# WeijingShi/Point-GNN

Hardware: AMD Instinct MI355X
Metric: KITTI-shaped frames/sec (car_auto_T3 inference: graph build + GNN, 20000 pts/frame, mean E1 602k) (higher is better)
Workload: dtype f32

## Files before the change

point-gnn_amd/csrc/edge_ws.h:

```cpp
#pragma once
#include "mlp_engine.h"
#include "ws_partition.h"

namespace pgnn {

#ifndef PGNN_WS_SCHED
#define PGNN_WS_SCHED 2
#endif

constexpr int kWsWaves = 8;
constexpr int kWsSchedInts = 2 + kWsMaxSlices * kWsMaxGroups;
constexpr int kWsStampTiles = 38;
constexpr int kWsStampStride = 8 + 4 * kWsStampTiles;

struct EdgeWsArgs {
  const float *P, *Q;
  int ldv4;
  const int32_t *edges;
  int64_t n_edges;
  const int32_t *n_dev;
  const float *wp;
  int nt;
  int relu_from;
  float *out;
  int64_t ldo;
  int num_segments;
  int sorted;
  int xcds;
  int prio;
  long long *ts;
  int32_t *sched;
  int pool_pct;
  int chunk;
  int groups;
  int tile0[kWsMaxGroups + 1];
  int wg0[kWsMaxGroups + 1];
  int balanced;
  int n_wg[kWsMaxGroups];
  short swg0[kWsMaxSlices][kWsMaxGroups + 1];
  short sbase[kWsMaxSlices][kWsMaxGroups];
  float *rows_out;
  int64_t ld_rows;
  float *h1_out;
  const int32_t *nv_dev;
};

__device__ __forceinline__ float opaque_inf() {
  float inf;
  asm("v_mov_b32 %0, 0x7f800000" : "=v"(inf));
  return inf;
}
__device__ __forceinline__ float max_nc(float a, float b, float inf) {
  return __builtin_amdgcn_fmed3f(a, b, inf);
}

typedef float v2f __attribute__((ext_vector_type(2)));
__device__ __forceinline__ v2f pk_sub(v2f a, v2f b) {
  v2f d;
  asm("v_pk_add_f32 %0, %1, %2 neg_lo:[0,1] neg_hi:[0,1]"
      : "=v"(d)
      : "v"(a), "v"(b));
  return d;
}

template <int CTRL>
__device__ __forceinline__ float dpp_mov(float x) {
  return __int_as_float(
      __builtin_amdgcn_update_dpp(0, __float_as_int(x), CTRL, 0xF, 0xF, false));
}

template <int NTG>
__device__ __forceinline__ float ws_v(const v4f (&v)[NTG], int i) {
  return i < 4 * NTG ? v[i >> 2][i & 3] : kFloatLowest;
}

template <int NTG, class ARGS>
__device__ __forceinline__ void ws_flush(const ARGS &a, const float *bias_lds,
                                         int t0, int lane, int d,
                                         const v4f (&v)[NTG], bool whole,
                                         float inf) {
  if (d < 0 || d >= a.num_segments) return;
  int zero;
  asm volatile("s_mov_b32 %0, 0" : "=s"(zero));
  const int n = (lane & 15) + zero, g = lane >> 4;
  const bool b0 = n & 1, b1 = n & 2, b2 = n & 4, b3 = n & 8;
  float A[16], B[8], C[4], D[2];
#pragma unroll
  for (int j = 0; j < 16; ++j) {
    if (2 * j < 4 * NTG) {
      const float x0 = ws_v<NTG>(v, 2 * j), x1 = ws_v<NTG>(v, 2 * j + 1);
      A[j] = max_nc(b0 ? x1 : x0, dpp_mov<0xB1>(b0 ? x0 : x1), inf);
    } else {
      A[j] = kFloatLowest;
    }
  }
#pragma unroll
  for (int k = 0; k < 8; ++k)
    B[k] = max_nc(b1 ? A[2 * k + 1] : A[2 * k],
                  dpp_mov<0x4E>(b1 ? A[2 * k] : A[2 * k + 1]), inf);
#pragma unroll
  for (int l = 0; l < 4; ++l)
    C[l] = max_nc(b2 ? B[2 * l + 1] : B[2 * l],
                  __shfl_xor(b2 ? B[2 * l] : B[2 * l + 1], 4), inf);
#pragma unroll
  for (int m = 0; m < 2; ++m)
    D[m] = max_nc(b3 ? C[2 * m + 1] : C[2 * m],
                  __shfl_xor(b3 ? C[2 * m] : C[2 * m + 1], 8), inf);
  float *orow = a.out + (int64_t)d * a.ldo + 16 * t0;
#pragma unroll
  for (int m = 0; m < 2; ++m) {
    const int i = 16 * m + n;
    if (i < 4 * NTG) {
      const int c = 16 * (i >> 2) + 4 * g + (i & 3);
      float x = D[m] + bias_lds[c];
      if (16 * t0 + c >= a.relu_from) x = x > 0.0f ? x : 0.0f;
      if (whole)
        orow[c] = x;
      else
        atomic_max_f32(orow + c, x + 0.0f);
    }
  }
}

struct WsRun {
  int cur_d;
  bool left_closed;
  bool has;
};

template <int NTG, class ARGS>
__device__ __forceinline__ void ws_epilogue(const ARGS &a, const float *bias_lds,
                                            int t0, int lane,
                                            const v4f (&acc)[NTG],
                                            v4f (&carry)[NTG], unsigned starts,
                                            int my_d, WsRun &st, bool fin,
                                            int d_after, float inf) {
  const int n = lane & 15;
  int cur_d = st.cur_d;
  bool cur_left_closed = st.left_closed, cur_has = st.has;
  int pos = 0;
  if (!(starts & 1u)) {
    const int f = starts ? __builtin_ctz(starts) : 16;
    if (f == 16) {
#pragma unroll
      for (int t = 0; t < NTG; ++t)
#pragma unroll
        for (int r = 0; r < 4; ++r)
          carry[t][r] = max_nc(carry[t][r], acc[t][r], inf);
    } else {
      const bool in_run = n < f;
#pragma unroll
      for (int t = 0; t < NTG; ++t)
#pragma unroll
        for (int r = 0; r < 4; ++r)
          carry[t][r] =
              max_nc(carry[t][r], in_run ? acc[t][r] : kFloatLowest, inf);
    }
    cur_has = true;
    pos = f;
  }
  while (pos < 16) {
    if (cur_has)
      ws_flush<NTG>(a, bias_lds, t0, lane, cur_d, carry,
                    a.sorted && cur_left_closed &&
                        (!fin || d_after != cur_d),
                    inf);
    if (fin) break;
    const unsigned rest = starts & ~((2u << pos) - 1u);
    const int nextpos = rest ? __builtin_ctz(rest) : 16;
    const bool in_run = n >= pos && n < nextpos;
#pragma unroll
    for (int t = 0; t < NTG; ++t)
#pragma unroll
      for (int r = 0; r < 4; ++r)
        carry[t][r] = in_run ? acc[t][r] : kFloatLowest;
    cur_d = __builtin_amdgcn_readlane(my_d, pos);
    cur_left_closed = true;
    cur_has = true;
    pos = nextpos;
  }
  st.cur_d = cur_d;
  st.left_closed = cur_left_closed;
  st.has = cur_has;
}

}

#include "ws_sum.h"

namespace pgnn {

template <int KQ, int NTG, bool EMIT, bool ROWS = false, class POL = WsMax>
__device__ __forceinline__ void edge_ws_body(const EdgeWsArgs &a,
                                             const v4f *__restrict__ wl, int t0,
                                             const float *bias_lds,
                                             int64_t tile_first,
                                             int64_t tile_last, int lane,
                                             long long *tsw, int &stamped,
                                             const int64_t E) {
  if (tile_first >= tile_last) return;
  const int n = lane & 15;
  const int64_t e_first = tile_first * 16;
  const int64_t e_end = tile_last * 16 < E ? tile_last * 16 : E;
  const v4f *__restrict__ P4 = reinterpret_cast<const v4f *>(a.P);
  const v4f *__restrict__ Q4 = reinterpret_cast<const v4f *>(a.Q);
  const int2 *__restrict__ e2 = reinterpret_cast<const int2 *>(a.edges);

  int cur_d = e_first > 0 ? a.edges[2 * (e_first - 1) + 1] : -1;
  int d_after = e_end < E ? a.edges[2 * e_end + 1] : -1;
  cur_d = __builtin_amdgcn_readfirstlane(cur_d);
  d_after = __builtin_amdgcn_readfirstlane(d_after);
  bool cur_left_closed = false, cur_has = false;
  constexpr float kIdentity = POL::kSum ? 0.0f : kFloatLowest;
  v4f carry[NTG];
#pragma unroll
  for (int t = 0; t < NTG; ++t)
    carry[t] = (v4f){kIdentity, kIdentity, kIdentity, kIdentity};

  const float inf = opaque_inf();
  bool nxt_ok = e_first + n < E;
  int2 nxt = e2[nxt_ok ? e_first + n : 0];
  for (int64_t tile = tile_first;; ++tile) {
    const bool fin = tile >= tile_last;
    const int64_t e0 = tile * 16;
    if (a.prio) __builtin_amdgcn_s_setprio(3);
    int lz;
    asm volatile("v_mov_b32 %0, %1" : "=v"(lz) : "v"(lane));
    const int g = lz >> 4;
    int lz1 = lz + 64 * 64, lz2 = lz + 128 * 64;
    asm volatile("" : "+v"(lz1));
    asm volatile("" : "+v"(lz2));
    const v4f *__restrict__ wfrag[3] = {wl + lz, wl + lz1, wl + lz2};
    long long *tst = nullptr;
    if (tsw && stamped < kWsStampTiles) tst = tsw + 8 + 4 * stamped++;
    if (tst) {
      __builtin_amdgcn_sched_barrier(0);
      const long long c = __builtin_readcyclecounter();
      if (lane == 0) tst[0] = c;
      __builtin_amdgcn_sched_barrier(0);
    }
    v4f acc[NTG];
    unsigned starts = 1u;
    int my_d = -1;
    if (fin) {
#pragma unroll
      for (int t = 0; t < NTG; ++t) acc[t] = (v4f){0.f, 0.f, 0.f, 0.f};
    } else {
    [[maybe_unused]] const int my_s = nxt_ok ? nxt.x : 0;
    my_d = nxt_ok ? nxt.y : -1;
    nxt_ok = tile + 1 < tile_last && e0 + 16 + n < E;
    nxt = e2[nxt_ok ? e0 + 16 + n : 0];
    v4f in[KQ];
    if constexpr (ROWS) {
      const int64_t row = e0 + n < E ? e0 + n : 0;
      const v4f *__restrict__ hr = P4 + row * a.ldv4 + g;
#pragma unroll
      for (int q = 0; q < KQ; ++q) in[q] = hr[4 * q];
      __builtin_amdgcn_sched_barrier(0);
    } else {
      const int dq = ((unsigned)my_d < (unsigned)a.num_segments) ? my_d : 0;
      const v4f *__restrict__ pr = P4 + (int64_t)my_s * a.ldv4 + g;
      const v4f *__restrict__ qr = Q4 + (int64_t)dq * a.ldv4 + g;
      v4f pq[KQ];
#pragma unroll
      for (int q = 0; q < KQ; ++q) {
#ifdef PGNN_WS_ABL_NO_GATHER
        in[q] = pr[0];
        pq[q] = qr[0];
#else
        in[q] = pr[4 * q];
        pq[q] = qr[4 * q];
#endif
      }
      __builtin_amdgcn_sched_barrier(0);
#pragma unroll
      for (int q = 0; q < KQ; ++q) {
        const v2f lo = pk_sub((v2f){in[q][0], in[q][1]}, (v2f){pq[q][0], pq[q][1]});
        const v2f hi = pk_sub((v2f){in[q][2], in[q][3]}, (v2f){pq[q][2], pq[q][3]});
        in[q][0] = max_nc(lo[0], 0.0f, inf);
        in[q][1] = max_nc(lo[1], 0.0f, inf);
        in[q][2] = max_nc(hi[0], 0.0f, inf);
        in[q][3] = max_nc(hi[1], 0.0f, inf);
      }
    }
    if constexpr (EMIT) {
      if (a.h1_out && t0 == 0 && e0 + n < E) {
        v4f *hrow = reinterpret_cast<v4f *>(a.h1_out) + (e0 + n) * a.ldv4 + g;
#pragma unroll
        for (int q = 0; q < KQ; ++q) hrow[4 * q] = in[q];
      }
    }
    __builtin_amdgcn_sched_barrier(0);
    if (tst) {
      const long long c = __builtin_readcyclecounter();
      if (lane == 0) tst[1] = c;
      __builtin_amdgcn_sched_barrier(0);
    }
    __builtin_amdgcn_s_setprio(0);
    {
      v4f w[2][NTG];
#pragma unroll
      for (int t = 0; t < NTG; ++t) {
        acc[t] = (v4f){0.f, 0.f, 0.f, 0.f};
        w[0][t] = wfrag[0][t * 64];
      }
      __builtin_amdgcn_sched_barrier(0);
#pragma unroll
      for (int q = 0; q < KQ; ++q) {
        __builtin_amdgcn_s_waitcnt(0xC07F);
        __builtin_amdgcn_sched_barrier(0);
        if (q + 1 < KQ) {
#pragma unroll
          for (int t = 0; t < NTG; ++t)
#ifdef PGNN_WS_ABL_NO_LDS
            w[(q + 1) & 1][t] = w[q & 1][t];
#else
            w[(q + 1) & 1][t] = wfrag[((q + 1) * NTG + t) >> 6]
                                     [(((q + 1) * NTG + t) & 63) * 64];
#endif
        }
#pragma unroll
        for (int s = 0; s < 4; ++s)
#pragma unroll
          for (int t = 0; t < NTG; ++t)
            acc[t] = __builtin_amdgcn_mfma_f32_16x16x4f32(
                w[q & 1][t][s], in[q][s], acc[t], 0, 0, 0);
#if PGNN_WS_SCHED == 2
#pragma unroll
        for (int t = 0; t < NTG; ++t) {
          __builtin_amdgcn_sched_group_barrier(0x8 , 3, 0);
          if (q + 1 < KQ)
            __builtin_amdgcn_sched_group_barrier(0x100 , 1, 0);
        }
        __builtin_amdgcn_sched_group_barrier(0x8 , NTG, 0);
#else
        if (q + 1 < KQ)
          __builtin_amdgcn_sched_group_barrier(0x100 , NTG, 0);
        __builtin_amdgcn_sched_group_barrier(0x8 , 4 * NTG, 0);
#endif
        __builtin_amdgcn_sched_barrier(0);
      }
    }
    if (tst) {
      const long long c = __builtin_readcyclecounter();
      if (lane == 0) tst[2] = c;
      __builtin_amdgcn_sched_barrier(0);
    }
    if constexpr (EMIT) {
      const int64_t row = e0 + n;
      if (row < E) {
        float *dstp = a.rows_out + row * a.ld_rows + 16 * t0 + 4 * g;
#pragma unroll
        for (int t = 0; t < NTG; ++t) {
          const v4f bb = *reinterpret_cast<const v4f *>(bias_lds + 16 * t + 4 * g);
          v4f y;
#pragma unroll
          for (int r = 0; r < 4; ++r) {
            float x = acc[t][r] + bb[r];
            if (16 * (t0 + t) + 4 * g + r >= a.relu_from) x = x > 0.0f ? x : 0.0f;
            y[r] = x;
          }
          *reinterpret_cast<v4f *>(dstp + 16 * t) = y;
        }
      }
    }
    if (a.prio) __builtin_amdgcn_s_setprio(3);
    const int up = __shfl_up(my_d, 1);
    const int prev = n == 0 ? cur_d : up;
    starts = (unsigned)(__ballot(my_d != prev) & 0xFFFFull);
    }
    WsRun st = {cur_d, cur_left_closed, cur_has};
    if constexpr (POL::kSum)
      ws_epilogue_sum<NTG>(a, bias_lds, t0, lane, acc, carry, starts, my_d, st,
                           fin, d_after, inf);
    else
      ws_epilogue<NTG>(a, bias_lds, t0, lane, acc, carry, starts, my_d, st, fin,
                       d_after, inf);
    cur_d = st.cur_d;
    cur_left_closed = st.left_closed;
    cur_has = st.has;
    if (fin) break;
    if (tst) {
      __builtin_amdgcn_sched_barrier(0);
      const long long c = __builtin_readcyclecounter();
      if (lane == 0) tst[3] = c;
    }
  }
  __builtin_amdgcn_s_setprio(0);
}


struct WsWho {
  int grp, t0, ntg;
  int64_t wi, nw;
};
__device__ __forceinline__ WsWho ws_who_balanced(const EdgeWsArgs &a, int slice,
                                                 int local, int wave) {
  int grp = 0;
  while (grp + 1 < a.groups && local >= a.swg0[slice][grp + 1]) ++grp;
  WsWho w;
  w.grp = grp;
  w.t0 = a.tile0[grp];
  w.ntg = a.tile0[grp + 1] - w.t0;
  w.nw = (int64_t)a.n_wg[grp] * kWsWaves;
  w.wi = (int64_t)(a.sbase[slice][grp] + local - a.swg0[slice][grp]) * kWsWaves +
         wave;
  return w;
}


template <int PER, class V, class ARGS, class MAP>
__device__ __forceinline__ void ws_stage(const ARGS &a, V *wl, int n_frag,
                                         MAP src_frag, size_t bias_at, int t0,
                                         int ntg, float *bias_lds, int wave,
                                         int lane) {
  const V *src = reinterpret_cast<const V *>(a.wp);
  V tmp[PER];
#pragma unroll
  for (int i = 0; i < PER; ++i) {
    const int f = wave + i * kWsWaves;
    tmp[i] = src[src_frag(f < n_frag ? f : 0) * 64 + lane];
  }
  __builtin_amdgcn_sched_barrier(0);
#pragma unroll
  for (int i = 0; i < PER; ++i) {
    const int f = wave + i * kWsWaves;
    if (f < n_frag) wl[(size_t)f * 64 + lane] = tmp[i];
  }
  if ((int)threadIdx.x < 16 * ntg)
    bias_lds[threadIdx.x] = a.wp[bias_at + 16 * t0 + threadIdx.x];
}

__device__ __forceinline__ int64_t ws_edge_count(int64_t cap,
                                                 const int32_t *n_dev) {
  if (n_dev) {
    const int64_t nd = *n_dev;
    cap = nd < cap ? nd : cap;
  }
  return cap;
}

__device__ __forceinline__ int ws_group(const EdgeWsArgs &a, int slice,
                                        int local, int wave) {
  if (a.balanced) return ws_who_balanced(a, slice, local, wave).grp;
  int grp = 0;
  while (grp + 1 < a.groups && local >= a.wg0[grp + 1]) ++grp;
  return grp;
}

struct WsShare {
  int64_t first, last, nw, wi;
};
__device__ __forceinline__ WsShare ws_share(const EdgeWsArgs &a, int grp,
                                            int slice, int local, int wave,
                                            int64_t n_wt) {
  WsShare s;
  s.first = n_wt * slice / a.xcds;
  s.last = n_wt * (slice + 1) / a.xcds;
  s.nw = (int64_t)(a.wg0[grp + 1] - a.wg0[grp]) * kWsWaves;
  s.wi = (int64_t)(local - a.wg0[grp]) * kWsWaves + wave;
  if (a.balanced) {
    const WsWho w = ws_who_balanced(a, slice, local, wave);
    s.first = 0;
    s.last = n_wt;
    s.nw = w.nw;
    s.wi = w.wi;
  }
  return s;
}

__device__ __forceinline__ int64_t ws_pool_size(int64_t span, const int32_t *sched,
                                                int pool_pct, int least,
                                                int64_t nw) {
  int64_t pool = sched ? span * pool_pct / 100 : 0;
  if (span - pool < least * nw) pool = 0;
  return pool;
}

__device__ __forceinline__ int ws_pool_claim(int32_t *counter, int chunk,
                                             int lane) {
  int c = 0;
  if (lane == 0)
    c = __hip_atomic_fetch_add(counter, chunk, __ATOMIC_RELAXED,
                               __HIP_MEMORY_SCOPE_AGENT);
  return __builtin_amdgcn_readfirstlane(c);
}

__device__ __forceinline__ void ws_pool_rearm(int32_t *sched, int n_counters,
                                              int lane) {
  if (sched && lane == 0) {
    const int total = (int)gridDim.x * kWsWaves;
    const int done = __hip_atomic_fetch_add(&sched[1], 1, __ATOMIC_ACQ_REL,
                                            __HIP_MEMORY_SCOPE_AGENT);
    if (done == total - 1) {
      for (int i = 0; i < n_counters; ++i)
        __hip_atomic_store(&sched[2 + i], 0, __ATOMIC_RELAXED,
                           __HIP_MEMORY_SCOPE_AGENT);
      __hip_atomic_store(&sched[1], 0, __ATOMIC_RELEASE,
                         __HIP_MEMORY_SCOPE_AGENT);
    }
  }
}

template <int KQ, int NTMAX, bool EMIT = false, bool ROWS = false,
          class POL = WsMax>
__global__ __launch_bounds__(64 * kWsWaves) void edge_ws_kernel(EdgeWsArgs a) {
  extern __shared__ __attribute__((aligned(16))) char smem[];
  v4f *wl = reinterpret_cast<v4f *>(smem);
  float *bias_lds = reinterpret_cast<float *>(wl + KQ * NTMAX * 64);
  const int lane = threadIdx.x & 63;
  const int wave = __builtin_amdgcn_readfirstlane(threadIdx.x >> 6);
  const int slice = blockIdx.x % a.xcds;
  const int local = blockIdx.x / a.xcds;
  const long long rt_entry = a.ts ? (long long)__builtin_amdgcn_s_memrealtime() : 0;
  const int grp = ws_group(a, slice, local, wave);
  const int t0 = a.tile0[grp];
  const int ntg = a.tile0[grp + 1] - t0;
  {
    const v4f *__restrict__ src = reinterpret_cast<const v4f *>(a.wp);
    constexpr int PER = (KQ * NTMAX + kWsWaves - 1) / kWsWaves;
    const int n_frag = KQ * ntg;
    v4f tmp[PER];
#pragma unroll
    for (int i = 0; i < PER; ++i) {
      const int f = wave + i * kWsWaves;
      const int fc = f < n_frag ? f : 0;
      const int q = fc / ntg, t = fc - q * ntg;
      tmp[i] = src[((size_t)q * a.nt + t0 + t) * 64 + lane];
    }
    __builtin_amdgcn_sched_barrier(0);
#pragma unroll
    for (int i = 0; i < PER; ++i) {
      const int f = wave + i * kWsWaves;
      if (f < n_frag) wl[(size_t)f * 64 + lane] = tmp[i];
    }
    if ((int)threadIdx.x < 16 * ntg)
      bias_lds[threadIdx.x] =
          a.wp[(size_t)KQ * a.nt * 256 + 16 * t0 + threadIdx.x];
  }
  __syncthreads();
  const int64_t n_edges = ws_edge_count(a.n_edges, a.n_dev);
  const WsShare s = ws_share(a, grp, slice, local, wave, (n_edges + 15) / 16);
  int64_t span = s.last - s.first;
  const int64_t pool = ws_pool_size(span, a.sched, a.pool_pct, 4, s.nw);
  span -= pool;
  const int64_t pool_first = s.first + span;
  int64_t tile_first = s.first + span * s.wi / s.nw;
  int64_t tile_last = s.first + span * (s.wi + 1) / s.nw;
  long long *tsw = nullptr;
  if (a.ts) {
    tsw = a.ts + ((int64_t)blockIdx.x * kWsWaves + wave) * kWsStampStride;
    if (lane == 0) {
      tsw[0] = __builtin_readcyclecounter();
      tsw[2] = __builtin_amdgcn_s_memrealtime();
      tsw[4] = tile_last - tile_first;
      tsw[5] = ntg + 100 * slice;
      tsw[6] = rt_entry;
    }
  }
  int stamped = 0;
  int32_t *counter = a.sched ? a.sched + 2 + slice * kWsMaxGroups + grp : nullptr;
  for (;;) {
    if (ntg == NTMAX)
      edge_ws_body<KQ, NTMAX, EMIT, ROWS, POL>(a, wl, t0, bias_lds, tile_first,
                                          tile_last, lane, tsw, stamped,
                                          n_edges);
    else
      edge_ws_body<KQ, NTMAX - 1, EMIT, ROWS, POL>(a, wl, t0, bias_lds, tile_first,
                                              tile_last, lane, tsw, stamped,
                                              n_edges);
    if (pool == 0) break;
    const int c = ws_pool_claim(counter, a.chunk, lane);
    if (c >= pool) break;
    tile_first = pool_first + c;
    tile_last = tile_first + a.chunk < s.last ? tile_first + a.chunk : s.last;
  }
  if (tsw && lane == 0) {
    tsw[1] = __builtin_readcyclecounter();
    tsw[3] = __builtin_amdgcn_s_memrealtime();
    tsw[7] = stamped;
  }
  if (a.sched && lane == 0) {
    const int total = (int)gridDim.x * kWsWaves;
    const int done = __hip_atomic_fetch_add(&a.sched[1], 1, __ATOMIC_ACQ_REL,
                                            __HIP_MEMORY_SCOPE_AGENT);
    if (done == total - 1) {
      for (int i = 0; i < a.xcds * kWsMaxGroups; ++i)
        __hip_atomic_store(&a.sched[2 + i], 0, __ATOMIC_RELAXED,
                           __HIP_MEMORY_SCOPE_AGENT);
      __hip_atomic_store(&a.sched[1], 0, __ATOMIC_RELEASE,
                         __HIP_MEMORY_SCOPE_AGENT);
    }
  }
}

}
```

point-gnn_amd/csrc/gnn.hip:

```cpp
#include <atomic>

#include "mlp_engine.h"
#include "edge_ws.h"
#include "edge_ws_split.h"
#include "pool_ws.h"
#include "pool_split.h"
#include "pool_ws_f16.h"

namespace pgnn {
int g_mlp_blocks_per_cu = 4;
int g_edge_msub = 0;
int g_pool_msub = 0;
int g_mlp_pool_pct = 12;
int g_ws_xcds = 8;
int g_ws_prio = 1;
int g_f16_pool = 1;
int g_b16_force = 0;
int g_ws_pool_pct = 0;
int g_ws_chunk = 2;
int g_ws_balance = 1;
int g_ws_reserve = 0;
void *g_mlp_ts = nullptr;
int g_mlp_debug = 0;
}
// ... 1988 lines not shown
  }
  a.c = c;
  a.xyz = xyz;
  a.wx = wx;
  a.n = n_vertices;
  a.n_dev = dk.dev;
  a.P = P;
  a.Q = Q;
  a.ld_pq = ld_pq;
  a.agg = agg;
  a.ld_agg = ld_agg;
  a.ld_tile = lds_ld(16 * pl.kq);
  a.ld_scratch = scratch_ld;
  return 0;
}

int pre_edge_impl(
    const float *h, int64_t ld_h, int32_t c, const float *xyz,
    const pgnn_fc_layer *offset_layers, int32_t n_offset_layers,
    const pgnn_fc_layer *p_layer, const float *wx, int64_t n_vertices, float *P,
    float *Q, int64_t ld_pq, float *agg, int64_t ld_agg, hipStream_t stream,
    const Dyn &dk) {
  PGNN_REQUIRE(n_vertices >= 0 && c > 0 && ld_h >= c && n_offset_layers >= 0 &&
                   n_offset_layers <= PGNN_MAX_LAYERS && p_layer,
               PGNN_E_INVALID, "vertex_pre_edge: bad argument");
  if (n_vertices == 0) return 0;
  PGNN_REQUIRE(h && xyz && wx && P && Q && (!agg || ld_agg > 0), PGNN_E_INVALID,
               "vertex_pre_edge: null pointer");
  ChainDev off;
  LayerDev pl;
  PreEdgeArgs a;
  const int rc = plan_pre_edge("vertex_pre_edge", c, xyz, offset_layers,
                               n_offset_layers, p_layer, wx, n_vertices, P, Q,
                               ld_pq, agg, ld_agg, dk, 0, off, pl, a);
  if (rc) return rc;
  a.h = h;
  a.ld_h = ld_h;
  const size_t lds =
      (size_t)16 * (a.ld_tile + a.ld_scratch + lds_ld(16 * pl.nt)) * 4;
  PGNN_REQUIRE(lds <= 160 * 1024, PGNN_E_UNSUPPORTED,
               "vertex_pre_edge: layer too wide for the LDS tile");
  g_vertex_lds[0][dk.dev ? 1 : 0] = (int64_t)lds;
  return launch_lds(
      dk.dev ? vertex_pre_edge_kernel<true> : vertex_pre_edge_kernel<false>,
      dim3((unsigned)dyn_grid_tiles(dk, n_vertices)), dim3(64 * kRowsWaves), lds,
      stream, off, pl, a);
}
}

namespace {
int plan_front(const float *x, int64_t ld_x, int32_t nx,
               const pgnn_fc_layer *front_layers, int32_t n_front,
               const float *residual, int64_t ld_res, float *y, int64_t ld_y,
               Plan &pf, FrontArgs &f) {
  PGNN_REQUIRE(x && y && nx > 0 && ld_x >= nx, PGNN_E_INVALID,
               "fused vertex stage: bad front input");
  int rc = make_plan(front_layers, n_front, nx, pf);
  if (rc) return rc;
  const int nt_last = pf.chain.l[n_front - 1].nt;
  PGNN_REQUIRE(nt_last <= kMaxTilesPerPass, PGNN_E_UNSUPPORTED,
               "fused vertex stage: front chain wider than 320");
  PGNN_REQUIRE(ld_y >= 16 * nt_last && (!residual || ld_res >= 16 * nt_last),
               PGNN_E_INVALID,
               "fused vertex stage: ld_y / ld_res < padded front width");
  f.x = x;
  f.ldx = ld_x;
  f.nx = nx;
  f.res = residual;
  f.ldres = ld_res;
  f.y = y;
  f.ldy = ld_y;
  f.ld_buf = pf.tile_floats_per_row;
  f.ld_stage = lds_ld(16 * nt_last);
  f.ts = (long long *)g_mlp_ts;
  return 0;
}

int update_pre_edge_impl(
    const float *x, int64_t ld_x, int32_t nx, const pgnn_fc_layer *front_layers,
    int32_t n_front, const float *residual, int64_t ld_res, float *y,
    int64_t ld_y, int32_t c, const float *xyz,
    const pgnn_fc_layer *offset_layers, int32_t n_offset_layers,
    const pgnn_fc_layer *p_layer, const float *wx, int64_t n_vertices, float *P,
    float *Q, int64_t ld_pq, float *agg, int64_t ld_agg, hipStream_t stream,
    const Dyn &dk) {
  PGNN_REQUIRE(n_vertices >= 0 && c > 0 && n_offset_layers >= 0 &&
                   n_offset_layers <= PGNN_MAX_LAYERS && p_layer,
               PGNN_E_INVALID, "vertex_update_pre_edge: bad argument");
  if (n_vertices == 0) return 0;
  PGNN_REQUIRE(xyz && wx && P && Q && (!agg || ld_agg > 0) && agg != x,
               PGNN_E_INVALID, "vertex_update_pre_edge: null / aliased pointer");
  PGNN_REQUIRE(expected(dk, n_vertices) <= 32 * (int64_t)device_cu_count(),
               PGNN_E_UNSUPPORTED, "vertex_update_pre_edge: too many rows");
  Plan pf;
  FrontArgs f;
  int rc = plan_front(x, ld_x, nx, front_layers, n_front, residual, ld_res, y,
                      ld_y, pf, f);
  if (rc) return rc;
  PGNN_REQUIRE(16 * pf.chain.l[n_front - 1].nt >= c &&
                   16 * pf.chain.l[n_front - 1].nt < c + 16,
               PGNN_E_INVALID,
               "vertex_update_pre_edge: front chain must produce c features");
  ChainDev off;
  LayerDev pl;
  PreEdgeArgs a;
  rc = plan_pre_edge("vertex_update_pre_edge", c, xyz, offset_layers,
                     n_offset_layers, p_layer, wx, n_vertices, P, Q, ld_pq, agg,
                     ld_agg, dk, kMaxTilesPerPass, off, pl, a);
  if (rc) return rc;
  a.h = nullptr;
  a.ld_h = 0;
  if (f.ld_buf < a.ld_tile) f.ld_buf = a.ld_tile;
  if (f.ld_stage < lds_ld(16 * pl.nt)) f.ld_stage = lds_ld(16 * pl.nt);
  const size_t lds = (size_t)16 * (f.ld_buf + a.ld_scratch + f.ld_stage) * 4;
  PGNN_REQUIRE(lds <= 160 * 1024, PGNN_E_UNSUPPORTED,
               "vertex_update_pre_edge: layers too wide for the LDS tile");
  g_vertex_lds[1][dk.dev ? 1 : 0] = (int64_t)lds;
  return launch_lds(dk.dev ? vertex_update_pre_edge_kernel<true>
                           : vertex_update_pre_edge_kernel<false>,
                    dim3((unsigned)dyn_grid_tiles(dk, n_vertices)),
                    dim3(64 * kRowsWaves), lds, stream, pf.chain, f, off, pl, a);
}

int mlp2_impl(const float *x, int64_t ld_x, int32_t nx,
              const pgnn_fc_layer *front_layers, int32_t n_front,
              const float *residual, int64_t ld_res, float *y, int64_t ld_y,
              int32_t ny, const pgnn_fc_layer *back_layers, int32_t n_back,
              float *out, int64_t ld_out, int64_t n_rows, hipStream_t stream,
              const Dyn &dk) {
  PGNN_REQUIRE(n_rows >= 0 && ny > 0, PGNN_E_INVALID, "mlp2: bad sizes");
  if (n_rows == 0) return 0;
  PGNN_REQUIRE(out, PGNN_E_INVALID, "mlp2: null output");
  PGNN_REQUIRE(expected(dk, n_rows) <= 32 * (int64_t)device_cu_count(),
               PGNN_E_UNSUPPORTED, "mlp2: too many rows for the 16-row kernel");
  Plan pf;
  FrontArgs f;
  int rc = plan_front(x, ld_x, nx, front_layers, n_front, residual, ld_res, y,
                      ld_y, pf, f);
  if (rc) return rc;
  PGNN_REQUIRE(ny <= 16 * pf.chain.l[n_front - 1].nt, PGNN_E_INVALID,
               "mlp2: ny wider than the front chain's output");
  Plan pb;
  rc = make_plan(back_layers, n_back, ny, pb);
  if (rc) return rc;
  const int nt_out = pb.chain.l[n_back - 1].nt;
  PGNN_REQUIRE(nt_out <= kMaxTilesPerPass &&
                   pb.chain.l[0].kq <= kMaxTilesPerPass,
               PGNN_E_UNSUPPORTED, "mlp2: back chain wider than 320");
  PGNN_REQUIRE(ld_out >= 16 * nt_out, PGNN_E_INVALID,
               "mlp2: ld_out < padded output width");
  if (f.ld_buf < pb.tile_floats_per_row) f.ld_buf = pb.tile_floats_per_row;
  if (f.ld_stage < lds_ld(16 * nt_out)) f.ld_stage = lds_ld(16 * nt_out);
  RowsArgs ro = {};
  ro.nx = ny;
  ro.y = out;
  ro.ldy = ld_out;
  const size_t lds = (size_t)16 * (f.ld_buf + f.ld_stage) * 4;
  PGNN_REQUIRE(lds <= 160 * 1024, PGNN_E_UNSUPPORTED,
               "mlp2: layers too wide for the LDS tile");
  g_vertex_lds[2][dk.dev ? 1 : 0] = (int64_t)lds;
  return launch_lds(dk.dev ? vertex_mlp2_kernel<true> : vertex_mlp2_kernel<false>,
                    dim3((unsigned)dyn_grid_tiles(dk, n_rows)),
                    dim3(64 * kRowsWaves), lds, stream, pf.chain, f, pb.chain,
                    ro, n_rows, dk.dev);
}
}

extern "C" int pgnn_vertex_update_pre_edge_fwd(
    const float *x, int64_t ld_x, int32_t nx, const pgnn_fc_layer *front_layers,
    int32_t n_front, const float *residual, int64_t ld_res, float *y,
    int64_t ld_y, int32_t c, const float *xyz,
    const pgnn_fc_layer *offset_layers, int32_t n_offset_layers,
    const pgnn_fc_layer *p_layer, const float *wx, int64_t n_vertices, float *P,
    float *Q, int64_t ld_pq, float *agg, int64_t ld_agg, void *stream_) {
  PGNN_GUARD_BEGIN
  return update_pre_edge_impl(x, ld_x, nx, front_layers, n_front, residual,
                              ld_res, y, ld_y, c, xyz, offset_layers,
                              n_offset_layers, p_layer, wx, n_vertices, P, Q,
                              ld_pq, agg, ld_agg, (hipStream_t)stream_,
                              dyn_of(nullptr));
  PGNN_GUARD_END
}

extern "C" int pgnn_vertex_update_pre_edge_fwd_dyn(
    const float *x, int64_t ld_x, int32_t nx, const pgnn_fc_layer *front_layers,
    int32_t n_front, const float *residual, int64_t ld_res, float *y,
    int64_t ld_y, int32_t c, const float *xyz,
    const pgnn_fc_layer *offset_layers, int32_t n_offset_layers,
    const pgnn_fc_layer *p_layer, const float *wx, int64_t vertices_cap,
    float *P, float *Q, int64_t ld_pq, float *agg, int64_t ld_agg,
    const pgnn_dyn_count *n_vertices, void *stream_) {
  PGNN_GUARD_BEGIN
  PGNN_REQUIRE(n_vertices && n_vertices->dev, PGNN_E_INVALID,
               "vertex_update_pre_edge_dyn: null count");
  return update_pre_edge_impl(x, ld_x, nx, front_layers, n_front, residual,
                              ld_res, y, ld_y, c, xyz, offset_layers,
                              n_offset_layers, p_layer, wx, vertices_cap, P, Q,
                              ld_pq, agg, ld_agg, (hipStream_t)stream_,
                              dyn_of(n_vertices));
  PGNN_GUARD_END
}

extern "C" int pgnn_mlp2_fwd(const float *x, int64_t ld_x, int32_t nx,
                             const pgnn_fc_layer *front_layers, int32_t n_front,
                             const float *residual, int64_t ld_res, float *y,
                             int64_t ld_y, int32_t ny,
                             const pgnn_fc_layer *back_layers, int32_t n_back,
                             float *out, int64_t ld_out, int64_t n_rows,
                             void *stream_) {
  PGNN_GUARD_BEGIN
  return mlp2_impl(x, ld_x, nx, front_layers, n_front, residual, ld_res, y,
                   ld_y, ny, back_layers, n_back, out, ld_out, n_rows,
                   (hipStream_t)stream_, dyn_of(nullptr));
  PGNN_GUARD_END
}

extern "C" int pgnn_mlp2_fwd_dyn(const float *x, int64_t ld_x, int32_t nx,
                                 const pgnn_fc_layer *front_layers,
                                 int32_t n_front, const float *residual,
                                 int64_t ld_res, float *y, int64_t ld_y,
                                 int32_t ny, const pgnn_fc_layer *back_layers,
                                 int32_t n_back, float *out, int64_t ld_out,
                                 int64_t rows_cap, const pgnn_dyn_count *rows,
                                 void *stream_) {
  PGNN_GUARD_BEGIN
  PGNN_REQUIRE(rows && rows->dev, PGNN_E_INVALID, "mlp2_dyn: null count");
  return mlp2_impl(x, ld_x, nx, front_layers, n_front, residual, ld_res, y,
                   ld_y, ny, back_layers, n_back, out, ld_out, rows_cap,
                   (hipStream_t)stream_, dyn_of(rows));
  PGNN_GUARD_END
}

extern "C" int pgnn_vertex_pre_edge_fwd(
    const float *h, int64_t ld_h, int32_t c, const float *xyz,
    const pgnn_fc_layer *offset_layers, int32_t n_offset_layers,
    const pgnn_fc_layer *p_layer, const float *wx, int64_t n_vertices, float *P,
    float *Q, int64_t ld_pq, float *agg, int64_t ld_agg, void *stream_) {
  PGNN_GUARD_BEGIN
  return pre_edge_impl(h, ld_h, c, xyz, offset_layers, n_offset_layers, p_layer,
                       wx, n_vertices, P, Q, ld_pq, agg, ld_agg,
                       (hipStream_t)stream_, dyn_of(nullptr));
  PGNN_GUARD_END
}

extern "C" int pgnn_vertex_pre_edge_fwd_dyn(
    const float *h, int64_t ld_h, int32_t c, const float *xyz,
    const pgnn_fc_layer *offset_layers, int32_t n_offset_layers,
    const pgnn_fc_layer *p_layer, const float *wx, int64_t vertices_cap,
    float *P, float *Q, int64_t ld_pq, float *agg, int64_t ld_agg,
    const pgnn_dyn_count *n_vertices, void *stream_) {
  PGNN_GUARD_BEGIN
  PGNN_REQUIRE(n_vertices && n_vertices->dev, PGNN_E_INVALID,
               "vertex_pre_edge_dyn: null count");
  return pre_edge_impl(h, ld_h, c, xyz, offset_layers, n_offset_layers, p_layer,
                       wx, vertices_cap, P, Q, ld_pq, agg, ld_agg,
                       (hipStream_t)stream_, dyn_of(n_vertices));
  PGNN_GUARD_END
}

extern "C" int pgnn_kernel_occupancy(const char *kernel, int64_t lds_bytes,
                                     int32_t *vgprs, int32_t *scratch_bytes,
                                     int32_t *workgroups_per_cu,
                                     int64_t *lds_used) {
  PGNN_GUARD_BEGIN
  PGNN_REQUIRE(kernel && vgprs && scratch_bytes && workgroups_per_cu,
               PGNN_E_INVALID, "kernel_occupancy: null argument");
  const std::string name(kernel);
  const struct {
    const char *name;
    const void *fn[2];
  } table[3] = {
      {"vertex_pre_edge",
       {reinterpret_cast<const void *>(vertex_pre_edge_kernel<false>),
        reinterpret_cast<const void *>(vertex_pre_edge_kernel<true>)}},
      {"vertex_update_pre_edge",
       {reinterpret_cast<const void *>(vertex_update_pre_edge_kernel<false>),
        reinterpret_cast<const void *>(vertex_update_pre_edge_kernel<true>)}},
      {"vertex_mlp2",
       {reinterpret_cast<const void *>(vertex_mlp2_kernel<false>),
        reinterpret_cast<const void *>(vertex_mlp2_kernel<true>)}},
  };
  for (int i = 0; i < 3; ++i)
    for (int dyn = 0; dyn < 2; ++dyn) {
      if (name != std::string(table[i].name) + (dyn ? "_dyn" : "")) continue;
      if (lds_bytes < 0) lds_bytes = g_vertex_lds[i][dyn];
      PGNN_REQUIRE(lds_bytes >= 0 && lds_bytes <= 160 * 1024, PGNN_E_INVALID,
                   "kernel_occupancy: no launch of this kernel yet, or more "
                   "LDS than a CU has");
      if (lds_bytes) {
        const int rc = ensure_dynamic_lds(table[i].fn[dyn], (size_t)lds_bytes);
        if (rc) return rc;
      }
      hipFuncAttributes attr;
      PGNN_HIP(hipFuncGetAttributes(&attr, table[i].fn[dyn]));
      int blocks = 0;
      PGNN_HIP(hipOccupancyMaxActiveBlocksPerMultiprocessor(
          &blocks, table[i].fn[dyn], 64 * kRowsWaves, (size_t)lds_bytes));
      *vgprs = attr.numRegs;
      *scratch_bytes = (int32_t)attr.localSizeBytes;
      *workgroups_per_cu = blocks;
      if (lds_used) *lds_used = lds_bytes;
      return 0;
    }
  PGNN_REQUIRE(false, PGNN_E_INVALID, "kernel_occupancy: unknown kernel");
  return 0;
  PGNN_GUARD_END
}

extern "C" int pgnn_point_set_pooling_rows_fwd(
    const float *point_features, int32_t n_feat, const float *point_xyz,
    const int32_t *keypoint_indices, const int32_t *edges, int64_t n_edges,
    int32_t num_keypoints, const pgnn_fc_layer *layers, int32_t n_layers,
    int32_t edges_sorted, float *out, int64_t ld_out, float *const *acts_host,
    int64_t ld_last, void *stream_) {
  PGNN_GUARD_BEGIN
  hipStream_t stream = (hipStream_t)stream_;
  PGNN_REQUIRE(n_edges >= 0 && num_keypoints >= 0 && n_feat >= 0 && n_feat <= 13 &&
                   layers && acts_host,
               PGNN_E_INVALID, "point_set_pooling_rows: bad sizes");
  if (n_layers != 4) return PGNN_E_UNSUPPORTED;
  Plan p;
  int rc = make_plan(layers, n_layers, n_feat + 3, p);
  if (rc) return rc;
  const int out_cols = 16 * p.chain.l[n_layers - 1].nt;
  PGNN_REQUIRE(out && ld_out >= out_cols && ld_last >= out_cols && ld_last % 4 == 0,
               PGNN_E_INVALID, "point_set_pooling_rows: bad output");
  const int cus = ws_cus(stream);
  if (n_edges == 0 || num_keypoints == 0 || !pool_ws_applies(p, n_edges, cus))
    return PGNN_E_UNSUPPORTED;
  PGNN_REQUIRE(point_xyz && keypoint_indices && edges && (n_feat == 0 || point_features),
               PGNN_E_INVALID, "point_set_pooling_rows: null input");
  for (int i = 0; i < 4; ++i)
    PGNN_REQUIRE(acts_host[i] && (uintptr_t)acts_host[i] % 16 == 0, PGNN_E_INVALID,
                 "point_set_pooling_rows: activation buffers must be 16-byte "
                 "aligned");
  if (!(edges_sorted & 2)) {
    rc = fill_lowest(out, (int64_t)num_keypoints * ld_out, stream);
    if (rc) return rc;
  }
  PoolArgs pa = {point_features, n_feat, point_xyz, keypoint_indices, edges};
  SegArgs sa = {out, ld_out, num_keypoints, edges_sorted & 1};
  return launch_pool_ws(p, pa, n_edges, sa, cus, nullptr, stream, acts_host,
                        ld_last);
  PGNN_GUARD_END
}

extern "C" int pgnn_edge_mlp_scatter_max_rows_fwd(
    const float *P, const float *Q, int64_t ld_pq, int32_t width,
    const int32_t *edges, int64_t n_edges, int32_t num_vertices,
    const pgnn_fc_layer *layer, int32_t edges_sorted, float *out, int64_t ld_out,
    float *rows_out, int64_t ld_rows, float *h1_out, void *stream_) {
  PGNN_GUARD_BEGIN
  hipStream_t stream = (hipStream_t)stream_;
  PGNN_REQUIRE(n_edges >= 0 && num_vertices >= 0 && width > 0 && layer,
               PGNN_E_INVALID, "edge_mlp_rows: bad sizes");
  Plan p;
  int rc = make_plan(layer, 1, width, p);
  if (rc) return rc;
  PGNN_REQUIRE(ld_pq == 16 * p.chain.l[0].kq, PGNN_E_INVALID,
               "edge_mlp_rows: ld_pq must equal the padded width");
  const int out_cols = 16 * p.chain.l[0].nt;
  PGNN_REQUIRE(out && ld_out >= out_cols && rows_out && ld_rows >= out_cols &&
                   ld_rows % 4 == 0 && (uintptr_t)rows_out % 16 == 0,
               PGNN_E_INVALID, "edge_mlp_rows: bad output");
  const int cus = ws_cus(stream);
  if (n_edges == 0 || num_vertices == 0 || !edge_ws_applies(p, n_edges, cus))
    return PGNN_E_UNSUPPORTED;
  PGNN_REQUIRE(P && Q && edges, PGNN_E_INVALID, "edge_mlp_rows: null input");
  PGNN_REQUIRE(((uintptr_t)P % 16 == 0) && ((uintptr_t)Q % 16 == 0) &&
                   ((uintptr_t)h1_out % 16 == 0),
               PGNN_E_INVALID, "edge_mlp_rows: P/Q/H1 must be 16-byte aligned");
  if (!(edges_sorted & 2)) {
    rc = fill_lowest(out, (int64_t)num_vertices * ld_out, stream);
    if (rc) return rc;
  }
  EdgeArgs ea = {P, Q, ld_pq, edges};
  SegArgs sa = {out, ld_out, num_vertices, edges_sorted & 1};
  if (p.chain.l[0].nt == 19)
    return launch_edge_ws<19, 7>(p.chain.l[0], ea, n_edges, sa, cus, nullptr,
                                 stream, rows_out, ld_rows, h1_out);
  return launch_edge_ws<16, 8>(p.chain.l[0], ea, n_edges, sa, cus, nullptr, stream,
                               rows_out, ld_rows, h1_out);
  PGNN_GUARD_END
}

extern "C" int pgnn_offset_apply(const float *xyz, const float *delta,
                                 int64_t ld_delta, int64_t n_rows,
                                 const float *wx, float *xyz_out, float *Q,
                                 int64_t ld_q, void *stream_) {
  PGNN_GUARD_BEGIN
  hipStream_t stream = (hipStream_t)stream_;
  PGNN_REQUIRE(n_rows >= 0 && ld_q >= 3, PGNN_E_INVALID,
               "offset_apply: bad sizes");
  if (n_rows == 0) return 0;
  PGNN_REQUIRE(xyz && wx && Q && (!delta || ld_delta >= 3), PGNN_E_INVALID,
               "offset_apply: null input");
  const int64_t total = n_rows * ld_q;
  int64_t blocks = (total + 255) / 256;
  if (blocks > 8192) blocks = 8192;
  return launch_lds(offset_apply_kernel, dim3((unsigned)blocks), dim3(256), 0,
                    stream, xyz, delta, ld_delta, n_rows, wx, xyz_out, Q, ld_q);
  PGNN_GUARD_END
}
```

Before: 325.8.

## Software-pipeline edge gathers one tile ahead inside the MFMA K loop

Splits the edge work-sharing body into a rows variant and a gather variant. The gather variant prefetches the next tile's source and destination feature rows while the current tile's MFMAs run. It applies the ReLU(P−Q) difference lagged by a small ring of Q registers, steered with sched_group_barrier. This hides gather latency behind matrix math, at the cost of more live registers and tighter scheduling constraints. It also adds occupancy-query entries for the edge kernels.

```diff
diff --git a/point-gnn_amd/csrc/edge_ws.h b/point-gnn_amd/csrc/edge_ws.h
--- a/point-gnn_amd/csrc/edge_ws.h
+++ b/point-gnn_amd/csrc/edge_ws.h
@@ -190,8 +190,8 @@
 
 namespace pgnn {
 
-template <int KQ, int NTG, bool EMIT, bool ROWS = false, class POL = WsMax>
-__device__ __forceinline__ void edge_ws_body(const EdgeWsArgs &a,
+template <int KQ, int NTG, bool EMIT, class POL>
+__device__ __forceinline__ void edge_ws_rows_body(const EdgeWsArgs &a,
                                              const v4f *__restrict__ wl, int t0,
                                              const float *bias_lds,
                                              int64_t tile_first,
@@ -203,7 +203,6 @@
   const int64_t e_first = tile_first * 16;
   const int64_t e_end = tile_last * 16 < E ? tile_last * 16 : E;
   const v4f *__restrict__ P4 = reinterpret_cast<const v4f *>(a.P);
-  const v4f *__restrict__ Q4 = reinterpret_cast<const v4f *>(a.Q);
   const int2 *__restrict__ e2 = reinterpret_cast<const int2 *>(a.edges);
 
   int cur_d = e_first > 0 ? a.edges[2 * (e_first - 1) + 1] : -1;
@@ -246,42 +245,16 @@
 #pragma unroll
       for (int t = 0; t < NTG; ++t) acc[t] = (v4f){0.f, 0.f, 0.f, 0.f};
     } else {
-    [[maybe_unused]] const int my_s = nxt_ok ? nxt.x : 0;
     my_d = nxt_ok ? nxt.y : -1;
     nxt_ok = tile + 1 < tile_last && e0 + 16 + n < E;
     nxt = e2[nxt_ok ? e0 + 16 + n : 0];
     v4f in[KQ];
-    if constexpr (ROWS) {
+    {
       const int64_t row = e0 + n < E ? e0 + n : 0;
       const v4f *__restrict__ hr = P4 + row * a.ldv4 + g;
 #pragma unroll
       for (int q = 0; q < KQ; ++q) in[q] = hr[4 * q];
       __builtin_amdgcn_sched_barrier(0);
-    } else {
-      const int dq = ((unsigned)my_d < (unsigned)a.num_segments) ? my_d : 0;
-      const v4f *__restrict__ pr = P4 + (int64_t)my_s * a.ldv4 + g;
-      const v4f *__restrict__ qr = Q4 + (int64_t)dq * a.ldv4 + g;
-      v4f pq[KQ];
-#pragma unroll
-      for (int q = 0; q < KQ; ++q) {
-#ifdef PGNN_WS_ABL_NO_GATHER
-        in[q] = pr[0];
-        pq[q] = qr[0];
-#else
-        in[q] = pr[4 * q];
-        pq[q] = qr[4 * q];
-#endif
-      }
-      __builtin_amdgcn_sched_barrier(0);
-#pragma unroll
-      for (int q = 0; q < KQ; ++q) {
-        const v2f lo = pk_sub((v2f){in[q][0], in[q][1]}, (v2f){pq[q][0], pq[q][1]});
-        const v2f hi = pk_sub((v2f){in[q][2], in[q][3]}, (v2f){pq[q][2], pq[q][3]});
-        in[q][0] = max_nc(lo[0], 0.0f, inf);
-        in[q][1] = max_nc(lo[1], 0.0f, inf);
-        in[q][2] = max_nc(hi[0], 0.0f, inf);
-        in[q][3] = max_nc(hi[1], 0.0f, inf);
-      }
     }
     if constexpr (EMIT) {
       if (a.h1_out && t0 == 0 && e0 + n < E) {
@@ -387,6 +360,243 @@
     }
   }
   __builtin_amdgcn_s_setprio(0);
+}
+
+constexpr int kWsRoll = 3;
+#ifndef PGNN_WS_PKSUB
+#define PGNN_WS_PKSUB 1
+#endif
+
+__device__ __forceinline__ void ws_relu_diff(v4f &in, const v4f &pq, float inf) {
+#if PGNN_WS_PKSUB
+  const v2f lo = pk_sub((v2f){in[0], in[1]}, (v2f){pq[0], pq[1]});
+  const v2f hi = pk_sub((v2f){in[2], in[3]}, (v2f){pq[2], pq[3]});
+  in[0] = max_nc(lo[0], 0.0f, inf);
+  in[1] = max_nc(lo[1], 0.0f, inf);
+  in[2] = max_nc(hi[0], 0.0f, inf);
+  in[3] = max_nc(hi[1], 0.0f, inf);
+#else
+#pragma unroll
+  for (int r = 0; r < 4; ++r) in[r] = max_nc(in[r] - pq[r], 0.0f, inf);
+#endif
+}
+
+template <int KQ, int NTG, bool EMIT, class POL>
+__device__ __forceinline__ void edge_ws_gather_body(const EdgeWsArgs &a,
+                                             const v4f *__restrict__ wl, int t0,
+                                             const float *bias_lds,
+                                             int64_t tile_first,
+                                             int64_t tile_last, int lane,
+                                             long long *tsw, int &stamped,
+                                             const int64_t E) {
+  if (tile_first >= tile_last) return;
+  constexpr int R = kWsRoll;
+  static_assert(KQ > R, "the ring is shorter than the K loop");
+  const int n = lane & 15;
+  const int64_t e_first = tile_first * 16;
+  const int64_t e_end = tile_last * 16 < E ? tile_last * 16 : E;
+  const v4f *__restrict__ P4 = reinterpret_cast<const v4f *>(a.P);
+  const v4f *__restrict__ Q4 = reinterpret_cast<const v4f *>(a.Q);
+  const int2 *__restrict__ e2 = reinterpret_cast<const int2 *>(a.edges);
+
+  int cur_d = e_first > 0 ? a.edges[2 * (e_first - 1) + 1] : -1;
+  int d_after = e_end < E ? a.edges[2 * e_end + 1] : -1;
+  cur_d = __builtin_amdgcn_readfirstlane(cur_d);
+  d_after = __builtin_amdgcn_readfirstlane(d_after);
+  bool cur_left_closed = false, cur_has = false;
+  constexpr float kIdentity = POL::kSum ? 0.0f : kFloatLowest;
+  v4f carry[NTG];
+#pragma unroll
+  for (int t = 0; t < NTG; ++t)
+    carry[t] = (v4f){kIdentity, kIdentity, kIdentity, kIdentity};
+
+  const float inf = opaque_inf();
+  const bool young =
+      __builtin_amdgcn_readfirstlane(threadIdx.x >> 6) >= kWsWaves / 2;
+  if (a.prio == 2 && young) __builtin_amdgcn_s_setprio(1);
+  const bool first_ok = e_first + n < E;
+  const int2 first = e2[first_ok ? e_first + n : 0];
+  bool nxt_ok = tile_first + 1 < tile_last && e_first + 16 + n < E;
+  int2 nxt = e2[nxt_ok ? e_first + 16 + n : 0];
+  int my_d = first_ok ? first.y : -1;
+  v4f in[KQ];
+  v4f w[2][NTG];
+  {
+    const int g = lane >> 4;
+    const int my_s = first_ok ? first.x : 0;
+    const int dq = ((unsigned)my_d < (unsigned)a.num_segments) ? my_d : 0;
+    const v4f *__restrict__ pr = P4 + (int64_t)my_s * a.ldv4 + g;
+    const v4f *__restrict__ qr = Q4 + (int64_t)dq * a.ldv4 + g;
+    v4f pq[KQ];
+#pragma unroll
+    for (int q = 0; q < KQ; ++q) {
+      in[q] = pr[4 * q];
+      pq[q] = qr[4 * q];
+    }
+#pragma unroll
+    for (int t = 0; t < NTG; ++t) w[0][t] = wl[t * 64 + lane];
+    __builtin_amdgcn_sched_barrier(0);
+#pragma unroll
+    for (int q = 0; q < KQ; ++q) ws_relu_diff(in[q], pq[q], inf);
+  }
+  for (int64_t tile = tile_first;; ++tile) {
+    const bool fin = tile >= tile_last;
+    const int64_t e0 = tile * 16;
+    int lz;
+    asm volatile("v_mov_b32 %0, %1" : "=v"(lz) : "v"(lane));
+    const int g = lz >> 4;
+    int lz1 = lz + 64 * 64, lz2 = lz + 128 * 64;
+    asm volatile("" : "+v"(lz1));
+    asm volatile("" : "+v"(lz2));
+    const v4f *__restrict__ wfrag[3] = {wl + lz, wl + lz1, wl + lz2};
+    long long *tst = nullptr;
+    if (tsw && stamped < kWsStampTiles) tst = tsw + 8 + 4 * stamped++;
+    if (tst) {
+      __builtin_amdgcn_sched_barrier(0);
+      const long long c = __builtin_readcyclecounter();
+      if (lane == 0) tst[0] = c;
+      __builtin_amdgcn_sched_barrier(0);
+    }
+    v4f acc[NTG];
+    v4f pq[R];
+    unsigned starts = 1u;
+    int nx_d = -1;
+    if (fin) {
+#pragma unroll
+      for (int t = 0; t < NTG; ++t) acc[t] = (v4f){0.f, 0.f, 0.f, 0.f};
+#pragma unroll
+      for (int r = 0; r < R; ++r) pq[r] = (v4f){0.f, 0.f, 0.f, 0.f};
+    } else {
+    const int nx_s = nxt_ok ? nxt.x : 0;
+    nx_d = nxt_ok ? nxt.y : -1;
+    nxt_ok = tile + 2 < tile_last && e0 + 32 + n < E;
+    nxt = e2[nxt_ok ? e0 + 32 + n : 0];
+    const int dq = ((unsigned)nx_d < (unsigned)a.num_segments) ? nx_d : 0;
+    const v4f *__restrict__ pr = P4 + (int64_t)nx_s * a.ldv4 + g;
+    const v4f *__restrict__ qr = Q4 + (int64_t)dq * a.ldv4 + g;
+    if constexpr (EMIT) {
+      if (a.h1_out && t0 == 0 && e0 + n < E) {
+        v4f *hrow = reinterpret_cast<v4f *>(a.h1_out) + (e0 + n) * a.ldv4 + g;
+#pragma unroll
+        for (int q = 0; q < KQ; ++q) hrow[4 * q] = in[q];
+      }
+    }
+    __builtin_amdgcn_sched_barrier(0);
+    if (tst) {
+      const long long c = __builtin_readcyclecounter();
+      if (lane == 0) tst[1] = c;
+      __builtin_amdgcn_sched_barrier(0);
+    }
+    if (a.prio == 1) __builtin_amdgcn_s_setprio(0);
+    if (a.prio == 3) {
+      if ((tile - tile_first + (young ? 1 : 0)) & 1)
+        __builtin_amdgcn_s_setprio(1);
+      else
+        __builtin_amdgcn_s_setprio(0);
+    }
+#pragma unroll
+    for (int t = 0; t < NTG; ++t) acc[t] = (v4f){0.f, 0.f, 0.f, 0.f};
+#pragma unroll
+    for (int q = 0; q < KQ; ++q) {
+      __builtin_amdgcn_s_waitcnt(0xC07F);
+      __builtin_amdgcn_sched_barrier(0);
+      const bool ahead = q + 1 < KQ;
+      if (ahead) {
+#pragma unroll
+        for (int t = 0; t < NTG; ++t)
+          w[(q + 1) & 1][t] = wfrag[((q + 1) * NTG + t) >> 6]
+                                   [(((q + 1) * NTG + t) & 63) * 64];
+      }
+#pragma unroll
+      for (int s = 0; s < 4; ++s)
+#pragma unroll
+        for (int t = 0; t < NTG; ++t)
+          acc[t] = __builtin_amdgcn_mfma_f32_16x16x4f32(
+              w[q & 1][t][s], in[q][s], acc[t], 0, 0, 0);
+      if (q >= R) {
+        ws_relu_diff(in[q - R], pq[q % R], inf);
+        asm volatile("" : "+v"(in[q - R]));
+      }
+      in[q] = pr[4 * q];
+      pq[q % R] = qr[4 * q];
+#pragma unroll
+      for (int t = 0; t < NTG; ++t) {
+        __builtin_amdgcn_sched_group_barrier(0x8 , 3, 0);
+        if (ahead) __builtin_amdgcn_sched_group_barrier(0x100 , 1, 0);
+        if (q >= R && t >= NTG - (PGNN_WS_PKSUB ? 2 : 4))
+          __builtin_amdgcn_sched_group_barrier(0x2 , 2, 0);
+      }
+      __builtin_amdgcn_sched_group_barrier(0x8 , NTG, 0);
+      __builtin_amdgcn_sched_group_barrier(0x20 , 2, 0);
+      __builtin_amdgcn_sched_barrier(0);
+    }
+    if (tst) {
+      const long long c = __builtin_readcyclecounter();
+      if (lane == 0) tst[2] = c;
+      __builtin_amdgcn_sched_barrier(0);
+    }
+    if (a.prio == 1) __builtin_amdgcn_s_setprio(3);
+    const int up = __shfl_up(my_d, 1);
+    const int prev = n == 0 ? cur_d : up;
+    starts = (unsigned)(__ballot(my_d != prev) & 0xFFFFull);
+    }
+    WsRun st = {cur_d, cur_left_closed, cur_has};
+    if constexpr (POL::kSum)
+      ws_epilogue_sum<NTG>(a, bias_lds, t0, lane, acc, carry, starts, my_d, st,
+                           fin, d_after, inf);
+    else
+      ws_epilogue<NTG>(a, bias_lds, t0, lane, acc, carry, starts, my_d, st, fin,
+                       d_after, inf);
+    cur_d = st.cur_d;
+    cur_left_closed = st.left_closed;
+    cur_has = st.has;
+    if (fin) break;
+#pragma unroll
+    for (int t = 0; t < NTG; ++t) w[0][t] = wfrag[0][t * 64];
+#pragma unroll
+    for (int q = KQ - R; q < KQ; ++q) ws_relu_diff(in[q], pq[q % R], inf);
+    if constexpr (EMIT) {
+      const int64_t row = e0 + n;
+      if (row < E) {
+        float *dstp = a.rows_out + row * a.ld_rows + 16 * t0 + 4 * g;
+#pragma unroll
+        for (int t = 0; t < NTG; ++t) {
+          const v4f bb = *reinterpret_cast<const v4f *>(bias_lds + 16 * t + 4 * g);
+          v4f y;
+#pragma unroll
+          for (int r = 0; r < 4; ++r) {
+            float x = acc[t][r] + bb[r];
+            if (16 * (t0 + t) + 4 * g + r >= a.relu_from) x = x > 0.0f ? x : 0.0f;
+            y[r] = x;
+          }
+          *reinterpret_cast<v4f *>(dstp + 16 * t) = y;
+        }
+      }
+    }
+    my_d = nx_d;
+    if (tst) {
+      __builtin_amdgcn_sched_barrier(0);
+      const long long c = __builtin_readcyclecounter();
+      if (lane == 0) tst[3] = c;
+    }
+  }
+  __builtin_amdgcn_s_setprio(0);
+}
+
+template <int KQ, int NTG, bool EMIT, bool ROWS = false, class POL = WsMax>
+__device__ __forceinline__ void edge_ws_body(const EdgeWsArgs &a,
+                                             const v4f *__restrict__ wl, int t0,
+                                             const float *bias_lds,
+                                             int64_t tile_first,
+                                             int64_t tile_last, int lane,
+                                             long long *tsw, int &stamped,
+                                             const int64_t E) {
+  if constexpr (ROWS)
+    edge_ws_rows_body<KQ, NTG, EMIT, POL>(a, wl, t0, bias_lds, tile_first,
+                                          tile_last, lane, tsw, stamped, E);
+  else
+    edge_ws_gather_body<KQ, NTG, EMIT, POL>(a, wl, t0, bias_lds, tile_first,
+                                            tile_last, lane, tsw, stamped, E);
 }
 
 
diff --git a/point-gnn_amd/csrc/gnn.hip b/point-gnn_amd/csrc/gnn.hip
--- a/point-gnn_amd/csrc/gnn.hip
+++ b/point-gnn_amd/csrc/gnn.hip
@@ -2314,6 +2314,44 @@
       if (lds_used) *lds_used = lds_bytes;
       return 0;
     }
+  const struct {
+    const char *name;
+    const void *fn;
+    int kq, ntmax;
+  } ws[6] = {
+      {"edge_ws_19_7", reinterpret_cast<const void *>(edge_ws_kernel<19, 7>), 19, 7},
+      {"edge_ws_16_8", reinterpret_cast<const void *>(edge_ws_kernel<16, 8>), 16, 8},
+      {"edge_ws_19_7_rows",
+       reinterpret_cast<const void *>(edge_ws_kernel<19, 7, true>), 19, 7},
+      {"edge_ws_16_8_rows",
+       reinterpret_cast<const void *>(edge_ws_kernel<16, 8, true>), 16, 8},
+      {"edge_ws_19_7_sum",
+       reinterpret_cast<const void *>(edge_ws_kernel<19, 7, false, false, WsSum>),
+       19, 7},
+      {"edge_ws_16_8_sum",
+       reinterpret_cast<const void *>(edge_ws_kernel<16, 8, false, false, WsSum>),
+       16, 8},
+  };
+  for (int i = 0; i < 6; ++i) {
+    if (name != ws[i].name) continue;
+    if (lds_bytes < 0)
+      lds_bytes = (int64_t)ws[i].kq * ws[i].ntmax * 1024 +
+                  16 * ws[i].ntmax * sizeof(float);
+    PGNN_REQUIRE(lds_bytes <= 160 * 1024, PGNN_E_INVALID,
+                 "kernel_occupancy: more LDS than a CU has");
+    const int rc = ensure_dynamic_lds(ws[i].fn, (size_t)lds_bytes);
+    if (rc) return rc;
+    hipFuncAttributes attr;
+    PGNN_HIP(hipFuncGetAttributes(&attr, ws[i].fn));
+    int blocks = 0;
+    PGNN_HIP(hipOccupancyMaxActiveBlocksPerMultiprocessor(
+        &blocks, ws[i].fn, 64 * kWsWaves, (size_t)lds_bytes));
+    *vgprs = attr.numRegs;
+    *scratch_bytes = (int32_t)attr.localSizeBytes;
+    *workgroups_per_cu = blocks;
+    if (lds_used) *lds_used = lds_bytes;
+    return 0;
+  }
   PGNN_REQUIRE(false, PGNN_E_INVALID, "kernel_occupancy: unknown kernel");
   return 0;
   PGNN_GUARD_END
```

New measurement: 328.6, median of 6. About the same (+0.8%).
